# Alandroid/img-compression-mps

Measured on AMD Instinct MI355X. Metric: Mvoxels/s compress+reconstruct, 256^3 fp32, bond chi=64; SSIM vs ref, higher is better.
Workload: dtype f32

## Files before the change

### img-compression-mps_amd/csrc/gemm.hip

```cpp
#include <stdlib.h>

#include <algorithm>

#include "common.h"
#include "gemm_plan.h"

namespace {

using ndmps::f64x4;
using ndmps::load4_stream_f32;
typedef float f32x16 __attribute__((ext_vector_type(16)));

template <typename T>
struct Mfma;

template <>
struct Mfma<float> {
  static constexpr int MT = 32;
  static constexpr int KS = 2;
  static constexpr int NACC = 16;
  typedef f32x16 acc_t;
  static __device__ __forceinline__ acc_t mma(float a, float b, acc_t c) {
    return __builtin_amdgcn_mfma_f32_32x32x2f32(a, b, c, 0, 0, 0);
  }
  static __device__ __forceinline__ int acc_row(int reg, int lane) {
    return (reg & 3) + 8 * (reg >> 2) + 4 * (lane >> 5);
  }
  static __device__ __forceinline__ int acc_col(int lane) { return lane & 31; }
  static __device__ __forceinline__ int frag_idx(int lane) { return lane & 31; }
  static __device__ __forceinline__ int frag_k(int lane) { return lane >> 5; }
};

template <>
struct Mfma<double> {
  static constexpr int MT = 16;
  static constexpr int KS = 4;
  static constexpr int NACC = 4;
  typedef f64x4 acc_t;
  static __device__ __forceinline__ acc_t mma(double a, double b, acc_t c) {
    return __builtin_amdgcn_mfma_f64_16x16x4f64(a, b, c, 0, 0, 0);
  }
  static __device__ __forceinline__ int acc_row(int reg, int lane) { return (lane >> 4) + 4 * reg; }
  static __device__ __forceinline__ int acc_col(int lane) { return lane & 15; }
  static __device__ __forceinline__ int frag_idx(int lane) { return lane & 15; }
  static __device__ __forceinline__ int frag_k(int lane) { return lane >> 4; }
};

template <typename T>
struct alignas(sizeof(T) * 4) Quad {
  T v[4];
};

struct GemmIndex {
  const int64_t* a_row;
  const int64_t* a_col;
  const int64_t* c_row;
  const int64_t* c_col;
  int guarded;
};
inline int gemm_guarded_env() { return getenv("NDMPS_GEMM_GUARDED") ? 1 : 0; }

constexpr int kGemmMaxBatch = 64;
struct GemmBatchPtrs {
  const void* a[kGemmMaxBatch];
  const void* b[kGemmMaxBatch];
  void* c[kGemmMaxBatch];
};

template <typename T, int BM, int BN, int WAVES_M, int WAVES_N, bool TA, bool TB, bool VEC, bool IDX>
__device__ __forceinline__ void
gemm_body(int64_t M, int64_t N, int64_t K, const T* __restrict__ A, int64_t lda, const T* __restrict__ B, int64_t ldb,
          T* __restrict__ C, int64_t ldc, const GemmIndex& ix) {
  using MF = Mfma<T>;
  constexpr int BK = 16;
  constexpr int MT = MF::MT;
  constexpr int TM = BM / (WAVES_M * MT);
  constexpr int TN = BN / (WAVES_N * MT);
  constexpr int PAD = 4;
  constexpr int A_PER = BM * BK / 256, B_PER = BN * BK / 256;
  static_assert(WAVES_M * WAVES_N == 4, "4 waves per workgroup");
  static_assert(TM >= 1 && TN >= 1, "tile too small");
  constexpr bool VA = VEC && A_PER % 4 == 0, VB = VEC && B_PER % 4 == 0;

  __shared__ T As[BK][BM + PAD];
  __shared__ T Bs[BK][BN + PAD];

  const int tid = threadIdx.x;
  const int lane = tid & 63;
  const int wave = tid >> 6;
  const int wm = wave / WAVES_N;
  const int wn = wave % WAVES_N;
  const int64_t m0 = (int64_t)blockIdx.x * BM;
  const int64_t n0 = (int64_t)blockIdx.y * BN;

  typename MF::acc_t acc[TM][TN];
#pragma unroll
  for (int i = 0; i < TM; ++i)
#pragma unroll
    for (int j = 0; j < TN; ++j)
#pragma unroll
      for (int r = 0; r < MF::NACC; ++r) acc[i][j][r] = (T)0;

  T ra[A_PER], rb[B_PER];

  constexpr int kIdxK = 1024;
  __shared__ int64_t acol_s[(IDX && !TA && VEC) ? kIdxK : 1];
  int64_t arow_q[(A_PER / 4) > 0 ? (A_PER / 4) : 1];
  const bool idx_fast = IDX && !TA && VA && ix.a_row != nullptr && K <= kIdxK;
  if (IDX && !TA && VA) {
    if (idx_fast) {
      for (int64_t kk = tid; kk < K; kk += 256) acol_s[kk] = ix.a_col[kk];
#pragma unroll
      for (int i = 0; i < A_PER / 4; ++i) {
        const int m = (tid + 256 * i) / (BK / 4);
        arow_q[i] = m0 + m < M ? ix.a_row[m0 + m] : 0;
      }
      __syncthreads();
    }
  }

  const bool inner_a = VA && m0 + BM <= M && !ix.guarded, inner_b = VB && n0 + BN <= N && !ix.guarded;
  auto fetch_a = [&](int64_t k0) {
    if (VA && inner_a && k0 + BK <= K) {
#pragma unroll
      for (int i = 0; i < A_PER / 4; ++i) {
        const int e = tid + 256 * i;
        const T* src;
        if (TA) {
          src = A + (k0 + e / (BM / 4)) * lda + m0 + (e % (BM / 4)) * 4;
        } else {
          const int m = e / (BK / 4), k = (e % (BK / 4)) * 4;
          if (IDX && idx_fast) src = A + arow_q[i] + acol_s[k0 + k];
          else if (IDX && ix.a_row) src = A + ix.a_row[m0 + m] + ix.a_col[k0 + k];
          else src = A + (m0 + m) * lda + k0 + k;
        }
        const Quad<T> q = *reinterpret_cast<const Quad<T>*>(src);
#pragma unroll
        for (int j = 0; j < 4; ++j) ra[4 * i + j] = q.v[j];
      }
    } else if (VA) {
#pragma unroll
      for (int i = 0; i < A_PER / 4; ++i) {
        const int e = tid + 256 * i;
        Quad<T> q;
        q.v[0] = q.v[1] = q.v[2] = q.v[3] = (T)0;
        if (TA) {
          const int k = e / (BM / 4), m = (e % (BM / 4)) * 4;
          if (k0 + k < K && m0 + m < M) q = *reinterpret_cast<const Quad<T>*>(A + (k0 + k) * lda + m0 + m);
        } else {
          const int m = e / (BK / 4), k = (e % (BK / 4)) * 4;
          if (k0 + k < K && m0 + m < M) {
            if (IDX && idx_fast) q = *reinterpret_cast<const Quad<T>*>(A + arow_q[i] + acol_s[k0 + k]);
            else if (IDX && ix.a_row) q = *reinterpret_cast<const Quad<T>*>(A + ix.a_row[m0 + m] + ix.a_col[k0 + k]);
            else q = *reinterpret_cast<const Quad<T>*>(A + (m0 + m) * lda + k0 + k);
          }
        }
#pragma unroll
        for (int j = 0; j < 4; ++j) ra[4 * i + j] = q.v[j];
      }
    } else {
#pragma unroll
      for (int i = 0; i < A_PER; ++i) {
        const int e = tid + 256 * i;
        int m, k;
        if (TA) {
          k = e / BM;
          m = e % BM;
        } else {
          m = e / BK;
          k = e % BK;
        }
        const int64_t gk = k0 + k, gm = m0 + m;
        if (IDX && ix.a_row) ra[i] = (gk < K && gm < M) ? A[ix.a_row[gm] + ix.a_col[gk]] : (T)0;
        else ra[i] = (gk < K && gm < M) ? (TA ? A[gk * lda + gm] : A[gm * lda + gk]) : (T)0;
      }
    }
  };
  auto fetch_b = [&](int64_t k0) {
    if (VB && inner_b && k0 + BK <= K) {
#pragma unroll
      for (int i = 0; i < B_PER / 4; ++i) {
        const int e = tid + 256 * i;
        const T* src = TB ? B + (n0 + e / (BK / 4)) * ldb + k0 + (e % (BK / 4)) * 4
                          : B + (k0 + e / (BN / 4)) * ldb + n0 + (e % (BN / 4)) * 4;
        const Quad<T> q = *reinterpret_cast<const Quad<T>*>(src);
#pragma unroll
        for (int j = 0; j < 4; ++j) rb[4 * i + j] = q.v[j];
      }
    } else if (VB) {
#pragma unroll
      for (int i = 0; i < B_PER / 4; ++i) {
        const int e = tid + 256 * i;
        Quad<T> q;
        q.v[0] = q.v[1] = q.v[2] = q.v[3] = (T)0;
        if (TB) {
          const int n = e / (BK / 4), k = (e % (BK / 4)) * 4;
          if (k0 + k < K && n0 + n < N) q = *reinterpret_cast<const Quad<T>*>(B + (n0 + n) * ldb + k0 + k);
        } else {
          const int k = e / (BN / 4), n = (e % (BN / 4)) * 4;
          if (k0 + k < K && n0 + n < N) q = *reinterpret_cast<const Quad<T>*>(B + (k0 + k) * ldb + n0 + n);
        }
#pragma unroll
        for (int j = 0; j < 4; ++j) rb[4 * i + j] = q.v[j];
      }
    } else {
#pragma unroll
      for (int i = 0; i < B_PER; ++i) {
        const int e = tid + 256 * i;
        int n, k;
        if (TB) {
          n = e / BK;
          k = e % BK;
        } else {
          k = e / BN;
          n = e % BN;
        }
        const int64_t gk = k0 + k, gn = n0 + n;
        rb[i] = (gk < K && gn < N) ? (TB ? B[gn * ldb + gk] : B[gk * ldb + gn]) : (T)0;
      }
    }
  };
  auto commit = [&]() {
    if (VA) {
#pragma unroll
      for (int i = 0; i < A_PER / 4; ++i) {
        const int e = tid + 256 * i;
        if (TA) {
          const int k = e / (BM / 4), m = (e % (BM / 4)) * 4;
#pragma unroll
          for (int j = 0; j < 4; ++j) As[k][m + j] = ra[4 * i + j];
        } else {
          const int m = e / (BK / 4), k = (e % (BK / 4)) * 4;
#pragma unroll
          for (int j = 0; j < 4; ++j) As[k + j][m] = ra[4 * i + j];
        }
      }
    } else {
#pragma unroll
      for (int i = 0; i < A_PER; ++i) {
        const int e = tid + 256 * i;
        if (TA) As[e / BM][e % BM] = ra[i];
        else As[e % BK][e / BK] = ra[i];
      }
    }
    if (VB) {
#pragma unroll
      for (int i = 0; i < B_PER / 4; ++i) {
        const int e = tid + 256 * i;
        if (TB) {
          const int n = e / (BK / 4), k = (e % (BK / 4)) * 4;
#pragma unroll
          for (int j = 0; j < 4; ++j) Bs[k + j][n] = rb[4 * i + j];
        } else {
          const int k = e / (BN / 4), n = (e % (BN / 4)) * 4;
#pragma unroll
          for (int j = 0; j < 4; ++j) Bs[k][n + j] = rb[4 * i + j];
        }
      }
    } else {
#pragma unroll
      for (int i = 0; i < B_PER; ++i) {
        const int e = tid + 256 * i;
        if (TB) Bs[e % BK][e / BK] = rb[i];
        else Bs[e / BN][e % BN] = rb[i];
      }
    }
  };

  fetch_a(0);
  fetch_b(0);
  const int fi = MF::frag_idx(lane);
  const int fk = MF::frag_k(lane);
  for (int64_t k0 = 0; k0 < K; k0 += BK) {
    __syncthreads();
    commit();
    __syncthreads();
    if (k0 + BK < K) {
      fetch_a(k0 + BK);
      fetch_b(k0 + BK);
    }
#pragma unroll
    for (int kk = 0; kk < BK; kk += MF::KS) {
      T a[TM], b[TN];
#pragma unroll
      for (int i = 0; i < TM; ++i) a[i] = As[kk + fk][(wm * TM + i) * MT + fi];
#pragma unroll
      for (int j = 0; j < TN; ++j) b[j] = Bs[kk + fk][(wn * TN + j) * MT + fi];
#pragma unroll
      for (int i = 0; i < TM; ++i)
#pragma unroll
        for (int j = 0; j < TN; ++j) acc[i][j] = MF::mma(a[i], b[j], acc[i][j]);
    }
  }

  if constexpr (IDX && MF::MT == 32 && BM == 128 && BN == 128 && sizeof(T) == 4) {
    if (ix.c_row) {
      __shared__ float cstage[4][32][36];
      float (*st)[36] = cstage[wave];
      const int rl0 = lane >> 3, cl = (lane & 7) * 4;
      int64_t roff[TM][4], coff[TN][4];
#pragma unroll
      for (int j = 0; j < TN; ++j) {
        const int64_t col = n0 + (wn * TN + j) * MT + cl;
#pragma unroll
        for (int e = 0; e < 4; ++e) coff[j][e] = col + e < N ? ix.c_col[col + e] : -1;
      }
#pragma unroll
      for (int i = 0; i < TM; ++i)
#pragma unroll
        for (int ps = 0; ps < 4; ++ps) {
          const int64_t row = m0 + (wm * TM + i) * MT + rl0 + 8 * ps;
          roff[i][ps] = row < M ? ix.c_row[row] : -1;
        }
#pragma unroll
      for (int i = 0; i < TM; ++i)
#pragma unroll
        for (int j = 0; j < TN; ++j) {
#pragma unroll
          for (int r = 0; r < MF::NACC; ++r) st[MF::acc_row(r, lane)][MF::acc_col(lane)] = acc[i][j][r];
          __builtin_amdgcn_fence(__ATOMIC_RELEASE, "wavefront");
          __builtin_amdgcn_wave_barrier();
          __builtin_amdgcn_fence(__ATOMIC_ACQUIRE, "wavefront");
          const bool run = coff[j][0] >= 0 && coff[j][3] == coff[j][0] + 3 && coff[j][1] == coff[j][0] + 1 &&
                           coff[j][2] == coff[j][0] + 2;
#pragma unroll
          for (int ps = 0; ps < 4; ++ps) {
            const float4 v = *reinterpret_cast<const float4*>(&st[rl0 + 8 * ps][cl]);
            const int64_t ro = roff[i][ps];
            if (ro < 0) continue;
            if (run && ((ro + coff[j][0]) & 3) == 0) {
              *reinterpret_cast<float4*>(C + ro + coff[j][0]) = v;
            } else {
              if (coff[j][0] >= 0) C[ro + coff[j][0]] = v.x;
              if (coff[j][1] >= 0) C[ro + coff[j][1]] = v.y;
              if (coff[j][2] >= 0) C[ro + coff[j][2]] = v.z;
              if (coff[j][3] >= 0) C[ro + coff[j][3]] = v.w;
            }
          }
          __builtin_amdgcn_fence(__ATOMIC_RELEASE, "wavefront");
          __builtin_amdgcn_wave_barrier();
        }
      return;
    }
  }
  if (IDX && ix.c_row) {
    int64_t roff[TM][MF::NACC], coff[TN];
#pragma unroll
    for (int j = 0; j < TN; ++j) {
      const int64_t col = n0 + (wn * TN + j) * MT + MF::acc_col(lane);
      coff[j] = col < N ? ix.c_col[col] : -1;
    }
#pragma unroll
    for (int i = 0; i < TM; ++i)
#pragma unroll
      for (int r = 0; r < MF::NACC; ++r) {
        const int64_t row = m0 + (wm * TM + i) * MT + MF::acc_row(r, lane);
        roff[i][r] = row < M ? ix.c_row[row] : -1;
      }
#pragma unroll
    for (int i = 0; i < TM; ++i)
#pragma unroll
      for (int j = 0; j < TN; ++j)
#pragma unroll
        for (int r = 0; r < MF::NACC; ++r)
          if (roff[i][r] >= 0 && coff[j] >= 0) C[roff[i][r] + coff[j]] = acc[i][j][r];
    return;
  }
#pragma unroll
  for (int i = 0; i < TM; ++i)
#pragma unroll
    for (int j = 0; j < TN; ++j) {
      const int64_t col = n0 + (wn * TN + j) * MT + MF::acc_col(lane);
#pragma unroll
      for (int r = 0; r < MF::NACC; ++r) {
        const int64_t row = m0 + (wm * TM + i) * MT + MF::acc_row(r, lane);
        if (row < M && col < N) C[row * ldc + col] = acc[i][j][r];
      }
    }
}

template <typename T, int BM, int BN, int WAVES_M, int WAVES_N, bool TA, bool TB, bool VEC, bool IDX = false>
__global__ void __launch_bounds__(256, 2)
// ... 21 lines not shown
#define NDMPS_GEMM_LAUNCH(TA_, TB_, V_)                                                                            \
  do {                                                                                                              \
    if (bp)                                                                                                         \
      hipLaunchKernelGGL((gemm_batched_kernel<T, BM, BN, WAVES_M, WAVES_N, TA_, TB_, V_>), grid, block, 0, stream,  \
                         m, n, k, *bp, lda, ldb, ldc, gi);                                                          \
    else                                                                                                            \
      hipLaunchKernelGGL((gemm_kernel<T, BM, BN, WAVES_M, WAVES_N, TA_, TB_, V_>), grid, block, 0, stream, m, n, k,  \
                         A, lda, B, ldb, C, ldc, gi);                                                               \
  } while (0)
#define NDMPS_GEMM_TRANS(V_)                                     \
  do {                                                           \
    if (transA && transB) NDMPS_GEMM_LAUNCH(true, true, V_);     \
    else if (transA) NDMPS_GEMM_LAUNCH(true, false, V_);         \
    else if (transB) NDMPS_GEMM_LAUNCH(false, true, V_);         \
    else NDMPS_GEMM_LAUNCH(false, false, V_);                    \
  } while (0)
  if (plan.vec) NDMPS_GEMM_TRANS(true);
  else NDMPS_GEMM_TRANS(false);
#undef NDMPS_GEMM_TRANS
#undef NDMPS_GEMM_LAUNCH
  NDMPS_LAUNCH_CHECK();
  return NDMPS_OK;
}

template <typename T>
constexpr ndmps::GemmElem gemm_elem() {
  return sizeof(T) == 8 ? ndmps::GemmElem::F64 : ndmps::GemmElem::F32;
}

inline int64_t gemm_misalignment(const void* p) { return (int64_t)((uintptr_t)p % 64); }

template <typename T>
int gemm_check(int64_t m, int64_t n, int64_t k, const T* A, int64_t lda, int transA, const T* B,
               int64_t ldb, int transB, T* C, int64_t ldc) {
  NDMPS_REQUIRE(A && B && C, "NULL GEMM operand");
  const char* why = ndmps::gemm_refusal(gemm_elem<T>(), transA, transB, m, n, k, lda, ldb, ldc);
  NDMPS_REQUIRE(!why, "%s (m=%lld n=%lld k=%lld lda=%lld ldb=%lld ldc=%lld)", why, (long long)m, (long long)n,
                (long long)k, (long long)lda, (long long)ldb, (long long)ldc);
  return NDMPS_OK;
}

template <typename T>
int gemm_run(int transA, int transB, int64_t m, int64_t n, int64_t k, const T* A, int64_t lda, const T* B, int64_t ldb,
             T* C, int64_t ldc, ndmps_stream_t stream, const GemmBatchPtrs* bp, int batch) {
  if (bp) {
    A = static_cast<const T*>(bp->a[0]);
    B = static_cast<const T*>(bp->b[0]);
    C = static_cast<T*>(bp->c[0]);
  }
  NDMPS_TRY(gemm_check(m, n, k, A, lda, transA, B, ldb, transB, C, ldc));
  int64_t mis_a = gemm_misalignment(A), mis_b = gemm_misalignment(B), mis_c = gemm_misalignment(C);
  for (int z = 1; bp && z < batch; ++z) {
    mis_a |= gemm_misalignment(bp->a[z]);
    mis_b |= gemm_misalignment(bp->b[z]);
    mis_c |= gemm_misalignment(bp->c[z]);
  }
  const ndmps::GemmPlan plan = ndmps::gemm_plan(gemm_elem<T>(), transA, transB, m, n, k, lda, ldb, ldc, mis_a, mis_b,
                                                mis_c, gemm_guarded_env() != 0);
  if (plan.launches == 0) return NDMPS_OK;
  hipStream_t s = (hipStream_t)stream;
  if (bp) A = B = nullptr, C = nullptr;
#define NDMPS_GEMM_TILE(BM_, BN_, WM_, WN_)  \
  if (plan.bm == BM_ && plan.bn == BN_)      \
  return launch_gemm<T, BM_, BN_, WM_, WN_>(plan, transA, transB, m, n, k, A, lda, B, ldb, C, ldc, s, bp, batch)
  if constexpr (sizeof(T) == 4) {
    NDMPS_GEMM_TILE(128, 32, 4, 1);
    NDMPS_GEMM_TILE(64, 64, 2, 2);
    NDMPS_GEMM_TILE(128, 128, 2, 2);
  } else {
    NDMPS_GEMM_TILE(64, 16, 4, 1);
    NDMPS_GEMM_TILE(32, 32, 2, 2);
    NDMPS_GEMM_TILE(64, 64, 2, 2);
  }
#undef NDMPS_GEMM_TILE
  ndmps::set_error("no kernel for the planned tile %d x %d", plan.bm, plan.bn);
  return NDMPS_EINVAL;
}

int launch_gemm_indexed(const ndmps::GemmPlan& plan, int64_t m, int64_t n, int64_t k, const float* A, int64_t lda,
                        const float* B, int64_t ldb, float* C, int64_t ldc, const GemmIndex& ix, hipStream_t s,
                        const GemmBatchPtrs* bp, int batch) {
  const dim3 block(256);
  const dim3 grid((unsigned)plan.grid_x, (unsigned)plan.grid_y, (unsigned)batch);
#define NDMPS_GEMM_IDX(BM_, V_)                                                                                        \
  do {                                                                                                                  \
    if (bp)                                                                                                             \
      hipLaunchKernelGGL((gemm_batched_kernel<float, BM_, BM_, 2, 2, false, false, V_, true>), grid, block, 0, s, m, n,  \
                         k, *bp, lda, ldb, ldc, ix);                                                                    \
    else                                                                                                                \
      hipLaunchKernelGGL((gemm_kernel<float, BM_, BM_, 2, 2, false, false, V_, true>), grid, block, 0, s, m, n, k, A,    \
                         lda, B, ldb, C, ldc, ix);                                                                      \
  } while (0)
  if (plan.bm == 64) {
    if (plan.vec) NDMPS_GEMM_IDX(64, true);
    else NDMPS_GEMM_IDX(64, false);
  } else {
    if (plan.vec) NDMPS_GEMM_IDX(128, true);
    else NDMPS_GEMM_IDX(128, false);
  }
#undef NDMPS_GEMM_IDX
  NDMPS_LAUNCH_CHECK();
  return NDMPS_OK;
}

}

extern "C" int ndmps_sgemm(int transA, int transB, int64_t m, int64_t n, int64_t k, const float* d_A,
                           int64_t lda, const float* d_B, int64_t ldb, float* d_C, int64_t ldc,
                           ndmps_stream_t stream) {
  return gemm_run<float>(transA, transB, m, n, k, d_A, lda, d_B, ldb, d_C, ldc, stream, nullptr, 1);
}

extern "C" int ndmps_sgemm_indexed(int64_t m, int64_t n, int64_t k, const float* d_A, int64_t lda,
                                   const int64_t* d_a_row, const int64_t* d_a_col, int a_vec4, const float* d_B,
                                   int64_t ldb, float* d_C, int64_t ldc, const int64_t* d_c_row,
                                   const int64_t* d_c_col, ndmps_stream_t stream) {
  NDMPS_REQUIRE(m >= 0 && n >= 0 && k >= 0 && d_A && d_B && d_C, "bad indexed GEMM argument");
  NDMPS_REQUIRE((d_a_row == nullptr) == (d_a_col == nullptr) && (d_c_row == nullptr) == (d_c_col == nullptr),
                "offset tables come in (row, column) pairs");
  NDMPS_REQUIRE(ldb >= n && (d_a_row || lda >= k) && (d_c_row || ldc >= n), "leading dimension too small");
  const ndmps::GemmPlan plan = ndmps::gemm_plan_indexed(m, n, k, lda, ldb, d_a_row != nullptr, a_vec4 != 0,
                                                        gemm_misalignment(d_A), gemm_misalignment(d_B),
                                                        gemm_guarded_env() != 0);
  if (plan.launches == 0) return NDMPS_OK;
  GemmIndex ix{d_a_row, d_a_col, d_c_row, d_c_col, plan.guarded};
  return launch_gemm_indexed(plan, m, n, k, d_A, lda, d_B, ldb, d_C, ldc, ix, (hipStream_t)stream, nullptr, 1);
}

extern "C" int ndmps_dgemm(int transA, int transB, int64_t m, int64_t n, int64_t k, const double* d_A,
                           int64_t lda, const double* d_B, int64_t ldb, double* d_C, int64_t ldc,
                           ndmps_stream_t stream) {
  return gemm_run<double>(transA, transB, m, n, k, d_A, lda, d_B, ldb, d_C, ldc, stream, nullptr, 1);
}

namespace {
template <typename T>
int gemm_batched_check(int batch, const T* const* h_A, const T* const* h_B, T* const* h_C, GemmBatchPtrs& bp) {
  NDMPS_REQUIRE(batch >= 1 && batch <= kGemmMaxBatch && h_A && h_B && h_C, "batched GEMM: batch=%d outside [1, %d] or NULL array",
                batch, kGemmMaxBatch);
  for (int z = 0; z < batch; ++z) {
    NDMPS_REQUIRE(h_A[z] && h_B[z] && h_C[z], "batched GEMM: NULL operand %d", z);
    bp.a[z] = h_A[z];
    bp.b[z] = h_B[z];
    bp.c[z] = h_C[z];
  }
  return NDMPS_OK;
}
}

extern "C" int ndmps_gemm_batched_max(void) { return kGemmMaxBatch; }

extern "C" int ndmps_sgemm_batched(int batch, int transA, int transB, int64_t m, int64_t n, int64_t k,
                                   const float* const* h_A, int64_t lda, const float* const* h_B, int64_t ldb,
                                   float* const* h_C, int64_t ldc, ndmps_stream_t stream) {
  GemmBatchPtrs bp;
  NDMPS_TRY(gemm_batched_check(batch, h_A, h_B, h_C, bp));
  return gemm_run<float>(transA, transB, m, n, k, nullptr, lda, nullptr, ldb, nullptr, ldc, stream, &bp, batch);
}

extern "C" int ndmps_dgemm_batched(int batch, int transA, int transB, int64_t m, int64_t n, int64_t k,
                                   const double* const* h_A, int64_t lda, const double* const* h_B, int64_t ldb,
                                   double* const* h_C, int64_t ldc, ndmps_stream_t stream) {
  GemmBatchPtrs bp;
  NDMPS_TRY(gemm_batched_check(batch, h_A, h_B, h_C, bp));
  return gemm_run<double>(transA, transB, m, n, k, nullptr, lda, nullptr, ldb, nullptr, ldc, stream, &bp, batch);
}

extern "C" int ndmps_gemm_plan_query(int elem, int transA, int transB, int64_t m, int64_t n, int64_t k, int64_t lda,
                                     int64_t ldb, int64_t ldc, int64_t mis_a, int64_t mis_b, int64_t mis_c, int guarded,
                                     int64_t* h_out) {
  NDMPS_REQUIRE(h_out && elem >= 0 && elem <= 2, "bad GEMM plan query (elem=%d)", elem);
  NDMPS_REQUIRE(mis_a >= 0 && mis_b >= 0 && mis_c >= 0, "a misalignment is a byte count");
  const ndmps::GemmElem e = (ndmps::GemmElem)elem;
  const char* why = ndmps::gemm_refusal(e, transA, transB, m, n, k, lda, ldb, ldc);
// ... 127 lines not shown
```

### img-compression-mps_amd/csrc/tt.hip

```cpp
#include <math.h>
#include <stdlib.h>

#include <algorithm>
#include <vector>

#include "common.h"
#include "trunc.h"
#include "typed.h"

namespace {

constexpr double kCutoffFloor = 1e-6;
constexpr double kCutoffFloorF64 = 1e-8;
template <typename T>
constexpr double cutoff_floor() { return sizeof(T) == 8 ? kCutoffFloorF64 : kCutoffFloor; }
constexpr double kSweepEigTol = 1e-13;

inline double sweep_eig_tol(bool f64_storage = false) {
  const char* e = getenv("NDMPS_SWEEP_EIG_TOL");
  if (e) {
    const double v = atof(e);
    if (v >= 1e-16 && v <= 1e-6) return v;
  }
  return f64_storage ? 1e-15 : kSweepEigTol;
// ... 63 lines not shown
  const int64_t total = rows * k;
  for (int64_t e = (int64_t)blockIdx.x * 256 + threadIdx.x; e < total; e += (int64_t)gridDim.x * 256) {
    const int64_t r = e / k, c = e % k;
    const double sg = sigma[c];
    out[e] = ndmps::from_f64<T>(sg > 0.0 ? M[r * ldm + c] * pow(sg, power) : 0.0);
  }
}
template <typename T>
__device__ __forceinline__ void scale_rows_body(const double* __restrict__ M, int64_t k, int64_t n,
                                                const double* __restrict__ sigma, double power, T* __restrict__ out) {
  const int64_t total = k * n;
  for (int64_t e = (int64_t)blockIdx.x * 256 + threadIdx.x; e < total; e += (int64_t)gridDim.x * 256) {
    const double sg = sigma[e / n];
    out[e] = ndmps::from_f64<T>(sg > 0.0 ? M[e] * pow(sg, power) : 0.0);
  }
}

template <typename T>
__global__ void __launch_bounds__(256)
core_from_vectors_kernel(const double* __restrict__ V, int64_t n, int64_t k, T* __restrict__ core,
                         const int* __restrict__ rank_r, int64_t cap_r) {
  core_from_vectors_body(V, n, k, core, rank_r, cap_r);
}
template <typename T>
__global__ void __launch_bounds__(256)
scale_cols_to_f32_kernel(const double* __restrict__ M, int64_t rows, int64_t ldm, int64_t k,
                         const double* __restrict__ sigma, double power, T* __restrict__ out) {
  scale_cols_body(M, rows, ldm, k, sigma, power, out);
}
template <typename T>
__global__ void __launch_bounds__(256)
scale_rows_to_f32_kernel(const double* __restrict__ M, int64_t k, int64_t n, const double* __restrict__ sigma,
                         double power, T* __restrict__ out) {
  scale_rows_body(M, k, n, sigma, power, out);
}
__global__ void __launch_bounds__(256) sqrt_clamp_kernel(const double* __restrict__ w, int64_t n, double* s) {
  sqrt_clamp_body(w, n, s);
}

__global__ void __launch_bounds__(256)
scale_cols_sqrt_kernel(double* __restrict__ M, int64_t rows, int64_t cols, const double* __restrict__ w,
                       double rel_zero = 0.0) {
  const double zero = rel_zero * fmax(fmax(w[0], w[cols - 1]), 0.0);
  const int64_t total = rows * cols;
  for (int64_t e = (int64_t)blockIdx.x * 256 + threadIdx.x; e < total; e += (int64_t)gridDim.x * 256) {
    const double we = w[e % cols];
    M[e] *= we > zero ? sqrt(we) : 0.0;
  }
}

constexpr int kSmallBatch = 64;
struct BatchOps {
  const void* in[kSmallBatch];
  void* out[kSmallBatch];
};
template <typename T>
__global__ void __launch_bounds__(256) f32_to_f64_batched_kernel(BatchOps ops, int64_t n, double* __restrict__ y, int64_t y_stride) {
  f32_to_f64_body(static_cast<const T*>(ops.in[blockIdx.y]), n, y + (int64_t)blockIdx.y * y_stride);
}
template <typename T>
__global__ void __launch_bounds__(256)
core_from_vectors_batched_kernel(const double* __restrict__ V, int64_t v_stride, int64_t n, int64_t k, BatchOps ops,
                                 const int* __restrict__ rank_r, int64_t cap_r) {
  core_from_vectors_body(V + (int64_t)blockIdx.y * v_stride, n, k, static_cast<T*>(ops.out[blockIdx.y]),
                         rank_r ? rank_r + blockIdx.y : nullptr, cap_r);
}
__global__ void __launch_bounds__(256)
sqrt_clamp_batched_kernel(const double* __restrict__ w, int64_t stride, int64_t n, double* __restrict__ sg) {
  sqrt_clamp_body(w + (int64_t)blockIdx.y * stride, n, sg + (int64_t)blockIdx.y * stride);
}
template <typename T>
__global__ void __launch_bounds__(256)
scale_cols_to_f32_batched_kernel(const double* __restrict__ M, int64_t m_stride, int64_t rows, int64_t ldm, int64_t k,
                                 const double* __restrict__ sigma, int64_t s_stride, double power, BatchOps ops) {
  scale_cols_body(M + (int64_t)blockIdx.y * m_stride, rows, ldm, k, sigma + (int64_t)blockIdx.y * s_stride, power,
                  static_cast<T*>(ops.out[blockIdx.y]));
}
template <typename T>
__global__ void __launch_bounds__(256)
scale_rows_to_f32_batched_kernel(const double* __restrict__ M, int64_t m_stride, int64_t k, int64_t n,
                                 const double* __restrict__ sigma, int64_t s_stride, double power, BatchOps ops) {
  scale_rows_body(M + (int64_t)blockIdx.y * m_stride, k, n, sigma + (int64_t)blockIdx.y * s_stride, power,
                  static_cast<T*>(ops.out[blockIdx.y]));
}

struct MergeRanks {
  int k_right[64];
  int k_here[64];
};

__global__ void __launch_bounds__(256)
merge_stage1_kernel(const double* __restrict__ Gtop, int64_t stride_top, int n_top, const double* __restrict__ W,
                    int64_t stride_w, int ldw, double* __restrict__ T, int64_t stride_t, int n_i, int n_right,
                    int d_i, MergeRanks rk) {
  const int b = blockIdx.y;
  const int k = rk.k_right[b];
  const int cols = d_i * k;
  const double* G = Gtop + (int64_t)b * stride_top;
  const double* Wb = W + (int64_t)b * stride_w;
  double* Tb = T + (int64_t)b * stride_t;
  const int reps = n_top / n_i;
  const int64_t total = (int64_t)n_i * cols;
  for (int64_t e = (int64_t)blockIdx.x * 256 + threadIdx.x; e < total; e += (int64_t)gridDim.x * 256) {
    const int r = (int)(e / cols), col = (int)(e % cols);
    const int bb = col / k, q = col % k;
    double acc = 0.0;
    for (int t = 0; t < reps; ++t) {
      const double* grow = G + (int64_t)(t * n_i + r) * n_top + t * n_i + bb * n_right;
      for (int c = 0; c < n_right; ++c) acc = fma(grow[c], Wb[(int64_t)c * ldw + q], acc);
    }
    Tb[e] = acc;
  }
}

__global__ void __launch_bounds__(256)
merge_stage2_kernel(const double* __restrict__ T, int64_t stride_t, const double* __restrict__ W, int64_t stride_w,
                    int ldw, double* __restrict__ Gout, int64_t stride_g, int n_right, int d_i, MergeRanks rk) {
  const int b = blockIdx.y;
  const int k = rk.k_right[b];
  const int n = d_i * k;
  const double* Tb = T + (int64_t)b * stride_t;
  const double* Wb = W + (int64_t)b * stride_w;
  double* Gb = Gout + (int64_t)b * stride_g;
  const int64_t total = (int64_t)n * n;
  for (int64_t e = (int64_t)blockIdx.x * 256 + threadIdx.x; e < total; e += (int64_t)gridDim.x * 256) {
    const int row = (int)(e / n), j = (int)(e % n);
    const int a = row / k, pp = row % k;
    double acc = 0.0;
    for (int c = 0; c < n_right; ++c) acc = fma(Wb[(int64_t)c * ldw + pp], Tb[(int64_t)(a * n_right + c) * n + j], acc);
    Gb[e] = acc;
  }
}

template <typename T>
__global__ void __launch_bounds__(256)
merge_basis_kernel(const double* __restrict__ Wr, int64_t stride_w, int ldw, const double* __restrict__ V,
                   int64_t stride_v, double* __restrict__ Wout, T* __restrict__ W32, int64_t stride_w32,
                   int n_right, int d_i, MergeRanks rk) {
  const int b = blockIdx.y;
  const int kr = rk.k_right[b], kh = rk.k_here[b];
  const int n = d_i * kr;
  const double* Wb = Wr + (int64_t)b * stride_w;
  const double* Vb = V + (int64_t)b * stride_v;
  double* Ob = Wout + (int64_t)b * stride_w;
  T* O32 = W32 ? W32 + (int64_t)b * stride_w32 : nullptr;
  const int64_t total = (int64_t)d_i * n_right * kh;
  for (int64_t e = (int64_t)blockIdx.x * 256 + threadIdx.x; e < total; e += (int64_t)gridDim.x * 256) {
    const int row = (int)(e / kh), pp = (int)(e % kh);
    const int a = row / n_right, c = row % n_right;
    double acc = 0.0;
    for (int q = 0; q < kr; ++q) acc = fma(Wb[(int64_t)c * ldw + q], Vb[(int64_t)(a * kr + q) * n + pp], acc);
    Ob[(int64_t)row * ldw + pp] = acc;
    if (O32) O32[(int64_t)row * kh + pp] = ndmps::from_f64<T>(acc);
  }
}

__global__ void merge_basis_init_kernel(double* __restrict__ W, int64_t stride_w) {
  W[(int64_t)blockIdx.x * stride_w] = 1.0;
}

__global__ void __launch_bounds__(256)
gather_rows_kernel(const float* __restrict__ W, int64_t rows, int64_t cols, const int32_t* __restrict__ perm,
                   float* __restrict__ out, int64_t w_stride = 0, int64_t out_stride = 0) {
  W += (int64_t)blockIdx.y * w_stride;
  out += (int64_t)blockIdx.y * out_stride;
  const int64_t total = rows * cols;
// ... 702 lines not shown
        NDMPS_LAUNCH_CHECK();
        NDMPS_TRY(ndmps_dgemm(0, 1, m, m, n, Ab, n, Ab, n, Gb(b), m, s));
      }
    }
    return NDMPS_OK;
  }

  const int* right_ranks(int i, int base) const {
    return lay.device_rank && ws.d_ranks && i + 1 < L ? ws.d_ranks + (int64_t)(i + 1) * batch + base : nullptr;
  }

  int site_core_and_carry(int i) {
    if (uniform_small() && uniform_kept()) {
      NDMPS_TRY(core_and_carry_uniform(i));
    } else {
      for (int b = 0; b < batch; ++b) NDMPS_TRY(core_and_carry_volume(i, b));
    }
    for (int b = 0; b < batch; ++b) {
      const int64_t m = cur_elems[b] / (h_dims[i] * chi_r[b]);
      std::swap(cur[b], nxt[b]);
      cur_elems[b] = m * kept[b];
      chi_r[b] = kept[b];
      h_bonds_out[(int64_t)b * (L + 1) + i] = kept[b];
    }
    return NDMPS_OK;
  }

  int core_and_carry_uniform(int i) {
    const int64_t n = h_dims[i] * chi_r[0], m = cur_elems[0] / n, small = eig_n[0], k = kept[0];
    BatchOps cores_out, carry_out;
    std::vector<T*> pcore(batch);
    for (int b = 0; b < batch; ++b) {
      pcore[b] = core(b, i);
      cores_out.out[b] = pcore[b];
      carry_out.out[b] = nxt[b];
    }
    if (n <= m) {
      hipLaunchKernelGGL(core_from_vectors_batched_kernel<T>, dim3(grid1d(k * n), batch), dim3(256), 0, s,
                         ws.V, sq, n, k, cores_out, right_ranks(i, 0), chi_r[0]);
      NDMPS_LAUNCH_CHECK();
      int rc = NDMPS_OK;
      const bool grouped = gemm_batched_T(batch, 1, m, k, n, cur.data(), pcore.data(), n, nxt.data(), s, &rc);
      NDMPS_TRY(rc);
      for (int b = 0; b < batch && !grouped; ++b)
        NDMPS_TRY(gemm_T(1, m, k, n, cur[b], pcore[b], n, nxt[b], ws.tws, lay.transpose_bytes, s));
      return NDMPS_OK;
    }
    const auto pv = strided(ws.V, sq), pa = strided(ws.A64, lay.wide_elems), pu = strided(ws.UtA, lay.wide_elems);
    hipLaunchKernelGGL(sqrt_clamp_batched_kernel, dim3(grid1d(small), batch), dim3(256), 0, s, ws.w,
                       lay.small_max, small, ws.sig);
    hipLaunchKernelGGL(scale_cols_to_f32_batched_kernel<T>, dim3(grid1d(m * k), batch), dim3(256), 0, s, ws.V,
                       sq, m, m, k, ws.sig, lay.small_max, 1.0, carry_out);
    NDMPS_LAUNCH_CHECK();
    NDMPS_TRY(ndmps_dgemm_batched(batch, 1, 0, k, n, m, pv.data(), m, pa.data(), n, pu.data(), n, s));
    hipLaunchKernelGGL(scale_rows_to_f32_batched_kernel<T>, dim3(grid1d(k * n), batch), dim3(256), 0, s,
                       ws.UtA, lay.wide_elems, k, n, ws.sig, lay.small_max, -1.0,
                       cores_out);
    NDMPS_LAUNCH_CHECK();
    return NDMPS_OK;
  }

  int core_and_carry_volume(int i, int b) {
    const int64_t n = h_dims[i] * chi_r[b], m = cur_elems[b] / n, small = eig_n[b], k = kept[b];
    const double* sigb = ws.sig + (int64_t)b * lay.small_max;
    if (n <= m) {
      hipLaunchKernelGGL(core_from_vectors_kernel<T>, dim3(grid1d(k * n)), dim3(256), 0, s, Vb(b), n, k,
                         core(b, i), right_ranks(i, b), chi_r[b]);
      NDMPS_LAUNCH_CHECK();
      return gemm_T(1, m, k, n, cur[b], core(b, i), n, nxt[b], ws.tws, lay.transpose_bytes, s);
    }
    hipLaunchKernelGGL(sqrt_clamp_kernel, dim3(grid1d(small)), dim3(256), 0, s, ws.w + (int64_t)b * lay.small_max,
                       small, ws.sig + (int64_t)b * lay.small_max);
    hipLaunchKernelGGL(scale_cols_to_f32_kernel<T>, dim3(grid1d(m * k)), dim3(256), 0, s, Vb(b), m, m, k, sigb,
                       1.0, nxt[b]);
    NDMPS_LAUNCH_CHECK();
    NDMPS_TRY(ndmps_dgemm(1, 0, k, n, m, Vb(b), m, ws.A64 + (int64_t)b * lay.wide_elems, n, ws.UtA, n, s));
    hipLaunchKernelGGL(scale_rows_to_f32_kernel<T>, dim3(grid1d(k * n)), dim3(256), 0, s, ws.UtA, k, n, sigb,
                       -1.0, core(b, i));
    NDMPS_LAUNCH_CHECK();
    return NDMPS_OK;
  }

  int finish() {
    for (int b = 0; b < batch; ++b)
      NDMPS_CHECK_HIP(hipMemcpyAsync(core(b, 0), cur[b], cur_elems[b] * sizeof(T), hipMemcpyDeviceToDevice, s));
    if (!lay.device_rank || L <= 1) {
      if (async) {
        ndmps::set_error("an asynchronous sweep needs ranks decided on the device (ndmps_tt_sweep_pads_cores) and more than one site");
        return NDMPS_EINVAL;
      }
      NDMPS_CHECK_HIP(hipStreamSynchronize(s));
      return NDMPS_OK;
    }
    const size_t n_i = (size_t)2 * L * batch, n_s = (size_t)L * batch * lay.spec_stride;
    std::vector<int> host_i(async ? 0 : n_i);
    std::vector<double> host_s(async ? 0 : n_s);
    if (async) NDMPS_REQUIRE(async->h_ranks && (async->h_spec || n_s == 0), "asynchronous sweep without its host buffers");
    int* dst_i = async ? async->h_ranks : host_i.data();
    double* dst_s = async ? async->h_spec : host_s.data();
    NDMPS_CHECK_HIP(hipMemcpyAsync(dst_i, ws.d_ranks, n_i * sizeof(int), hipMemcpyDeviceToHost, s));
    if (n_s) NDMPS_CHECK_HIP(hipMemcpyAsync(dst_s, ws.d_spec, n_s * sizeof(double), hipMemcpyDeviceToHost, s));
    if (async) return NDMPS_OK;
    NDMPS_CHECK_HIP(hipStreamSynchronize(s));
    return sweep_collect(batch, L, lay.spec_stride, dst_i, n_s ? dst_s : nullptr, h_bonds_out, h_spectra, h_spec_offsets);
  }
};

template <typename T>
int sweep_impl(int batch, T* const* h_dense, int L, const int64_t* h_dims, double cutoff, int64_t max_bond,
               T* const* h_cores, const int64_t* h_core_offsets, int64_t* h_bonds_out, double* h_spectra,
               const int64_t* h_spec_offsets, void* d_ws, int64_t ws_bytes, ndmps_stream_t stream,
               const SweepSource* src = nullptr, const SweepAsync* async = nullptr) {
  Sweep<T> sw{batch, h_dense, L, h_dims, cutoff, max_bond, h_cores, h_core_offsets, h_bonds_out, h_spectra,
              h_spec_offsets, d_ws, ws_bytes, (hipStream_t)stream, src, async};
  NDMPS_TRY(sw.prepare());
  int i = L - 1;
  if (sw.lay.merge_from < L) {
    NDMPS_TRY(sw.merged_run());
    i = sw.lay.merge_from - 1;
  }
  for (; i >= 1; --i) {
    NDMPS_TRY(sw.site_gram(i));
    NDMPS_TRY(sw.solve_site(i, true));
    NDMPS_TRY(sw.site_core_and_carry(i));
  }
  return sw.finish();
}
}

extern "C" int ndmps_tt_sweep_pads_cores(int L, const int64_t* h_dims, int64_t max_bond) {
  SweepLayout lay;
  if (!h_dims || sweep_layout(L, h_dims, max_bond, 1, lay) != NDMPS_OK) return 0;
  return lay.device_rank ? 1 : 0;
}

extern "C" int ndmps_tt_sweep_batched_f32(int batch, float* const* h_dense, int L, const int64_t* h_dims,
                                          double cutoff, int64_t max_bond, float* const* h_cores,
                                          const int64_t* h_core_offsets, int64_t* h_bonds_out,
                                          double* h_spectra, const int64_t* h_spec_offsets, void* d_ws,
                                          int64_t ws_bytes, ndmps_stream_t stream) {
  return sweep_impl<float>(batch, h_dense, L, h_dims, cutoff, max_bond, h_cores, h_core_offsets, h_bonds_out, h_spectra,
                           h_spec_offsets, d_ws, ws_bytes, stream);
}

extern "C" int64_t ndmps_tt_merge_columns(int L, const int64_t* h_dims, int64_t max_bond) {
  SweepLayout lay;
  if (!h_dims || sweep_layout(L, h_dims, max_bond, 1, lay) != NDMPS_OK) return 0;
  if (lay.merge_from >= L || (lay.numel / lay.merge_n) * lay.merge_w > lay.numel / 2) return 0;
  if (lay.merge_n < 64 || lay.numel / lay.merge_n < 256 || lay.merge_n % 4 != 0) return 0;
  return lay.merge_n;
}

extern "C" int ndmps_tt_sweep_batched_fused_f32(int batch, const float* const* h_volume, int L, const int64_t* h_dims,
                                                double cutoff, int64_t max_bond, float* const* h_cores,
                                                const int64_t* h_core_offsets, int64_t* h_bonds_out,
                                                double* h_spectra, const int64_t* h_spec_offsets,
                                                const int64_t* d_row_off, const int64_t* d_row_off_sorted,
                                                const int32_t* d_row_order, const int64_t* d_col_off,
                                                const int32_t* d_col_perm, int64_t n_cols, void* d_ws, int64_t ws_bytes,
                                                ndmps_stream_t stream) {
  NDMPS_REQUIRE(d_row_off && d_col_off && d_col_perm && n_cols >= 1, "NULL permutation table");
  SweepSource src{d_row_off, d_row_off_sorted ? d_row_off_sorted : d_row_off, d_row_off_sorted ? d_row_order : nullptr, d_col_off,
                  d_col_perm, n_cols};
  return retry_without_team([&]() {
    return sweep_impl<float>(batch, (float* const*)h_volume, L, h_dims, cutoff, max_bond, h_cores, h_core_offsets,
                             h_bonds_out, h_spectra, h_spec_offsets, d_ws, ws_bytes, stream, &src);
  });
}
// ... 278 lines not shown
```

Measured before the change: 42540.

## Double-buffer interior indexed GEMM tiles and batch final core copies into one kernel

Adds a fast path for full interior tiles of the indexed fp32 GEMM. It double-buffers LDS with register prefetch two tiles ahead, stages the next tile in the middle of the MFMA steps, and preloads the output row/column index tables into shared memory so the epilogue can use vectorised float4 scatter when the indices are contiguous. The LDS arrays are merged into one buffer that the epilogue staging reuses, and the column-index table moves to dynamic shared memory. In tt.hip, the per-batch device-to-device memcpys in finish() are replaced by a single batched copy kernel to cut launch overhead. The changes add considerable complexity and carry risks in LDS aliasing and in the alignment assumptions.

```diff
diff --git a/img-compression-mps_amd/csrc/gemm.hip b/img-compression-mps_amd/csrc/gemm.hip
--- a/img-compression-mps_amd/csrc/gemm.hip
+++ b/img-compression-mps_amd/csrc/gemm.hip
@@ -1,6 +1,7 @@
 #include <stdlib.h>
 
 #include <algorithm>
+#include <type_traits>
 
 #include "common.h"
 #include "gemm_plan.h"
@@ -59,6 +60,10 @@
   int guarded;
 };
 inline int gemm_guarded_env() { return getenv("NDMPS_GEMM_GUARDED") ? 1 : 0; }
+constexpr int kGemmIdxK = 1024;
+inline size_t gemm_acol_bytes(const GemmIndex& ix, bool vec, int64_t k) {
+  return ix.a_row && vec && k <= kGemmIdxK ? sizeof(int64_t) * (size_t)k : 0;
+}
 
 constexpr int kGemmMaxBatch = 64;
 struct GemmBatchPtrs {
@@ -82,8 +87,18 @@
   static_assert(TM >= 1 && TN >= 1, "tile too small");
   constexpr bool VA = VEC && A_PER % 4 == 0, VB = VEC && B_PER % 4 == 0;
 
-  __shared__ T As[BK][BM + PAD];
-  __shared__ T Bs[BK][BN + PAD];
+  constexpr bool kInterior = IDX && VA && VB && !TA && !TB && sizeof(T) == 4 && MT == 32;
+  constexpr bool kPatch = IDX && MT == 32 && BM == 128 && BN == 128 && sizeof(T) == 4;
+  constexpr int NBUF = kInterior ? 2 : 1;
+  constexpr int kTileElems = NBUF * BK * (BM + PAD + BN + PAD);
+  constexpr int kPatchElems = kPatch ? 4 * 2 * 32 * 36 : 0;
+  __shared__ __attribute__((aligned(16))) T smem[kTileElems > kPatchElems ? kTileElems : kPatchElems];
+  T (*As)[BM + PAD] = reinterpret_cast<T (*)[BM + PAD]>(smem);
+  T (*Bs)[BN + PAD] = reinterpret_cast<T (*)[BN + PAD]>(smem + NBUF * BK * (BM + PAD));
+  [[maybe_unused]] int64_t* crow_s = reinterpret_cast<int64_t*>(smem + kTileElems);
+  [[maybe_unused]] int64_t* ccol_s = crow_s + BM;
+  static_assert(!kPatch || (kTileElems * sizeof(T) % 8 == 0 && kTileElems * sizeof(T) + (BM + BN / 4) * 8 <= kPatchElems * sizeof(T)),
+                "the table offsets do not fit behind the operand tiles");
 
   const int tid = threadIdx.x;
   const int lane = tid & 63;
@@ -103,8 +118,8 @@
 
   T ra[A_PER], rb[B_PER];
 
-  constexpr int kIdxK = 1024;
-  __shared__ int64_t acol_s[(IDX && !TA && VEC) ? kIdxK : 1];
+  constexpr int kIdxK = kGemmIdxK;
+  extern __shared__ int64_t acol_s[];
   int64_t arow_q[(A_PER / 4) > 0 ? (A_PER / 4) : 1];
   const bool idx_fast = IDX && !TA && VA && ix.a_row != nullptr && K <= kIdxK;
   if (IDX && !TA && VA) {
@@ -267,37 +282,205 @@
     }
   };
 
-  fetch_a(0);
-  fetch_b(0);
   const int fi = MF::frag_idx(lane);
   const int fk = MF::frag_k(lane);
-  for (int64_t k0 = 0; k0 < K; k0 += BK) {
-    __syncthreads();
-    commit();
-    __syncthreads();
-    if (k0 + BK < K) {
-      fetch_a(k0 + BK);
-      fetch_b(k0 + BK);
-    }
-#pragma unroll
-    for (int kk = 0; kk < BK; kk += MF::KS) {
-      T a[TM], b[TN];
-#pragma unroll
-      for (int i = 0; i < TM; ++i) a[i] = As[kk + fk][(wm * TM + i) * MT + fi];
-#pragma unroll
-      for (int j = 0; j < TN; ++j) b[j] = Bs[kk + fk][(wn * TN + j) * MT + fi];
-#pragma unroll
-      for (int i = 0; i < TM; ++i)
-#pragma unroll
-        for (int j = 0; j < TN; ++j) acc[i][j] = MF::mma(a[i], b[j], acc[i][j]);
-    }
-  }
-
-  if constexpr (IDX && MF::MT == 32 && BM == 128 && BN == 128 && sizeof(T) == 4) {
+
+  bool interior = false;
+  int64_t c_roff[TM][4], c_col0[TN];
+  bool c_fast = false;
+  if constexpr (kInterior) {
+    constexpr int64_t kDenseLd = (int64_t)1 << 22;
+    interior = m0 + BM <= M && n0 + BN <= N && K >= BK && K % BK == 0 && K <= kIdxK && !ix.guarded && ldb <= kDenseLd &&
+               (ix.a_row || lda <= kDenseLd);
+    if (interior) {
+      constexpr int QA = A_PER / 4, QB = B_PER / 4, STEPS = BK / MF::KS;
+      const int nt = (int)(K / BK);
+      const int kq = (tid % (BK / 4)) * 4;
+      uint32_t aoff[QA], boff[QB];
+#pragma unroll
+      for (int i = 0; i < QA; ++i) aoff[i] = (uint32_t)((((tid + 256 * i) / (BK / 4)) * lda + kq) * sizeof(T));
+#pragma unroll
+      for (int i = 0; i < QB; ++i) {
+        const int e = tid + 256 * i;
+        boff[i] = (uint32_t)(((e / (BN / 4)) * ldb + (e % (BN / 4)) * 4) * sizeof(T));
+      }
+      static_assert(!kPatch || (BM <= 256 && (BM & (BM - 1)) == 0 && ((BN / 4) & (BN / 4 - 1)) == 0), "BM, BN / 4: powers of two");
+      [[maybe_unused]] int64_t c_req_row, c_req[4];
+      if constexpr (kPatch) {
+        if (ix.c_row) {
+          c_req_row = ix.c_row[m0 + (tid & (BM - 1))];
+#pragma unroll
+          for (int e = 0; e < 4; ++e) c_req[e] = ix.c_col[n0 + (tid & (BN / 4 - 1)) * 4 + e];
+        }
+      }
+      auto park_c = [&]() {
+        if constexpr (kPatch) {
+          if (ix.c_row) {
+            if (tid < BM) crow_s[tid] = c_req_row;
+            const bool run = c_req[1] == c_req[0] + 1 && c_req[2] == c_req[0] + 2 && c_req[3] == c_req[0] + 3;
+            if (tid < BN / 4) ccol_s[tid] = run ? c_req[0] : -1;
+          }
+        }
+      };
+      Quad<T> qa[2][QA], qb[2][QB];
+      auto load = [&](auto tabled, int t, Quad<T>* a, Quad<T>* b) {
+        if constexpr (decltype(tabled)::value) {
+          const int64_t ao = acol_s[t * BK + kq];
+#pragma unroll
+          for (int i = 0; i < QA; ++i) a[i] = *reinterpret_cast<const Quad<T>*>(A + arow_q[i] + ao);
+        } else {
+          const char* at = reinterpret_cast<const char*>(A + m0 * lda + (int64_t)t * BK);
+#pragma unroll
+          for (int i = 0; i < QA; ++i) a[i] = *reinterpret_cast<const Quad<T>*>(at + aoff[i]);
+        }
+        const char* bt = reinterpret_cast<const char*>(B + (int64_t)t * BK * ldb + n0);
+#pragma unroll
+        for (int i = 0; i < QB; ++i) b[i] = *reinterpret_cast<const Quad<T>*>(bt + boff[i]);
+      };
+      constexpr int LDA_S = BM + PAD, LDB_S = BN + PAD, B_AT = NBUF * BK * LDA_S;
+      const int stage_a0 = kq * LDA_S + tid / (BK / 4);
+      const int stage_b0 = B_AT + (tid / (BN / 4)) * LDB_S + (tid % (BN / 4)) * 4;
+      const int frag_a0 = fk * LDA_S + wm * TM * MT + fi;
+      const int frag_b0 = B_AT + fk * LDB_S + wn * TN * MT + fi;
+      auto here = [](int x) {
+        asm volatile("" : "+v"(x));
+        return x;
+      };
+      auto stage = [&](int buf, const Quad<T>* a, const Quad<T>* b) {
+        const int sa = here(stage_a0 + buf * BK * LDA_S), sb = here(stage_b0 + buf * BK * LDB_S);
+#pragma unroll
+        for (int i = 0; i < QA; ++i)
+#pragma unroll
+          for (int j = 0; j < 4; ++j) smem[sa + j * LDA_S + i * (256 / (BK / 4))] = a[i].v[j];
+#pragma unroll
+        for (int i = 0; i < QB; ++i)
+#pragma unroll
+          for (int j = 0; j < 4; ++j) smem[sb + i * (256 / (BN / 4)) * LDB_S + j] = b[i].v[j];
+      };
+      auto frag = [&](int fa, int fb, int kk, T* a, T* b) {
+#pragma unroll
+        for (int i = 0; i < TM; ++i) a[i] = smem[fa + kk * LDA_S + i * MT];
+#pragma unroll
+        for (int j = 0; j < TN; ++j) b[j] = smem[fb + kk * LDB_S + j * MT];
+      };
+      auto tile = [&](auto tabled, auto parity, auto steady, int t) {
+        constexpr int P = decltype(parity)::value;
+        constexpr bool STEADY = decltype(steady)::value;
+        if (STEADY || t + 2 < nt) load(tabled, t + 2, qa[P], qb[P]);
+        T a[2][TM], b[2][TN];
+        const int fa = here(frag_a0 + P * BK * LDA_S), fb = here(frag_b0 + P * BK * LDB_S);
+        frag(fa, fb, 0, a[0], b[0]);
+#pragma unroll
+        for (int s = 0; s < STEPS; ++s) {
+          if (s + 1 < STEPS) frag(fa, fb, (s + 1) * MF::KS, a[(s + 1) & 1], b[(s + 1) & 1]);
+#pragma unroll
+          for (int i = 0; i < TM; ++i)
+#pragma unroll
+            for (int j = 0; j < TN; ++j) acc[i][j] = MF::mma(a[s & 1][i], b[s & 1][j], acc[i][j]);
+          if (s == STEPS / 2 && (STEADY || t + 1 < nt)) stage(1 - P, qa[1 - P], qb[1 - P]);
+          __builtin_amdgcn_sched_barrier(0);
+        }
+        if (STEADY || t + 1 < nt) __syncthreads();
+      };
+      using Even = std::integral_constant<int, 0>;
+      using Odd = std::integral_constant<int, 1>;
+      auto run = [&](auto tabled) {
+        load(tabled, 0, qa[0], qb[0]);
+        if (nt > 1) load(tabled, 1, qa[1], qb[1]);
+        park_c();
+        stage(0, qa[0], qb[0]);
+        __syncthreads();
+        int t = 0;
+        for (; t + 3 < nt; t += 2) {
+          tile(tabled, Even(), std::true_type(), t);
+          tile(tabled, Odd(), std::true_type(), t + 1);
+        }
+        for (; t < nt; t += 2) {
+          tile(tabled, Even(), std::false_type(), t);
+          if (t + 1 < nt) tile(tabled, Odd(), std::false_type(), t + 1);
+        }
+        if constexpr (kPatch) {
+          if (ix.c_row) {
+            const int rl0 = lane >> 3, cl = (lane & 7) * 4;
+            c_fast = true;
+#pragma unroll
+            for (int j = 0; j < TN; ++j) {
+              c_col0[j] = ccol_s[((wn * TN + j) * MT + cl) / 4];
+              c_fast = c_fast && c_col0[j] >= 0;
+            }
+#pragma unroll
+            for (int i = 0; i < TM; ++i)
+#pragma unroll
+              for (int ps = 0; ps < 4; ++ps) {
+                c_roff[i][ps] = crow_s[(wm * TM + i) * MT + rl0 + 8 * ps];
+#pragma unroll
+                for (int j = 0; j < TN; ++j) c_fast = c_fast && ((c_roff[i][ps] + c_col0[j]) & 3) == 0;
+              }
+          }
+        }
+      };
+      if (ix.a_row) run(std::true_type());
+      else run(std::false_type());
+    }
+  }
+
+  if (!interior) {
+    fetch_a(0);
+    fetch_b(0);
+    for (int64_t k0 = 0; k0 < K; k0 += BK) {
+      __syncthreads();
+      commit();
+      __syncthreads();
+      if (k0 + BK < K) {
+        fetch_a(k0 + BK);
+        fetch_b(k0 + BK);
+      }
+#pragma unroll
+      for (int kk = 0; kk < BK; kk += MF::KS) {
+        T a[TM], b[TN];
+#pragma unroll
+        for (int i = 0; i < TM; ++i) a[i] = As[kk + fk][(wm * TM + i) * MT + fi];
+#pragma unroll
+        for (int j = 0; j < TN; ++j) b[j] = Bs[kk + fk][(wn * TN + j) * MT + fi];
+#pragma unroll
+        for (int i = 0; i < TM; ++i)
+#pragma unroll
+          for (int j = 0; j < TN; ++j) acc[i][j] = MF::mma(a[i], b[j], acc[i][j]);
+      }
+    }
+  }
+
+  if constexpr (kPatch) {
     if (ix.c_row) {
-      __shared__ float cstage[4][32][36];
-      float (*st)[36] = cstage[wave];
+      __shared__ int c_ok[4];
+      const bool wave_ok = __all(c_fast);
+      if (lane == 0) c_ok[wave] = wave_ok;
+      __syncthreads();
+      float (*st)[36] = reinterpret_cast<float (*)[36]>(smem + wave * (2 * 32 * 36));
       const int rl0 = lane >> 3, cl = (lane & 7) * 4;
+      if constexpr (kInterior) {
+        if (c_ok[0] && c_ok[1] && c_ok[2] && c_ok[3]) {
+          auto put = [&](int q) {
+#pragma unroll
+            for (int r = 0; r < MF::NACC; ++r)
+              st[(q & 1) * 32 + MF::acc_row(r, lane)][MF::acc_col(lane)] = acc[q / TN][q % TN][r];
+          };
+          put(0);
+#pragma unroll
+          for (int q = 0; q < TM * TN; ++q) {
+            __builtin_amdgcn_fence(__ATOMIC_RELEASE, "wavefront");
+            __builtin_amdgcn_wave_barrier();
+            __builtin_amdgcn_fence(__ATOMIC_ACQUIRE, "wavefront");
+            float4 v[4];
+#pragma unroll
+            for (int ps = 0; ps < 4; ++ps) v[ps] = *reinterpret_cast<const float4*>(&st[(q & 1) * 32 + rl0 + 8 * ps][cl]);
+            if (q + 1 < TM * TN) put(q + 1);
+#pragma unroll
+            for (int ps = 0; ps < 4; ++ps) *reinterpret_cast<float4*>(C + c_roff[q / TN][ps] + c_col0[q % TN]) = v[ps];
+          }
+          return;
+        }
+      }
       int64_t roff[TM][4], coff[TN][4];
 #pragma unroll
       for (int j = 0; j < TN; ++j) {
@@ -485,14 +668,15 @@
                         const GemmBatchPtrs* bp, int batch) {
   const dim3 block(256);
   const dim3 grid((unsigned)plan.grid_x, (unsigned)plan.grid_y, (unsigned)batch);
-#define NDMPS_GEMM_IDX(BM_, V_)                                                                                        \
-  do {                                                                                                                  \
-    if (bp)                                                                                                             \
-      hipLaunchKernelGGL((gemm_batched_kernel<float, BM_, BM_, 2, 2, false, false, V_, true>), grid, block, 0, s, m, n,  \
-                         k, *bp, lda, ldb, ldc, ix);                                                                    \
-    else                                                                                                                \
-      hipLaunchKernelGGL((gemm_kernel<float, BM_, BM_, 2, 2, false, false, V_, true>), grid, block, 0, s, m, n, k, A,    \
-                         lda, B, ldb, C, ldc, ix);                                                                      \
+  const size_t acol = gemm_acol_bytes(ix, plan.vec != 0, k);
+#define NDMPS_GEMM_IDX(BM_, V_)                                                                                          \
+  do {                                                                                                                    \
+    if (bp)                                                                                                               \
+      hipLaunchKernelGGL((gemm_batched_kernel<float, BM_, BM_, 2, 2, false, false, V_, true>), grid, block, acol, s, m, n, \
+                         k, *bp, lda, ldb, ldc, ix);                                                                      \
+    else                                                                                                                  \
+      hipLaunchKernelGGL((gemm_kernel<float, BM_, BM_, 2, 2, false, false, V_, true>), grid, block, acol, s, m, n, k, A,   \
+                         lda, B, ldb, C, ldc, ix);                                                                        \
   } while (0)
   if (plan.bm == 64) {
     if (plan.vec) NDMPS_GEMM_IDX(64, true);
diff --git a/img-compression-mps_amd/csrc/tt.hip b/img-compression-mps_amd/csrc/tt.hip
--- a/img-compression-mps_amd/csrc/tt.hip
+++ b/img-compression-mps_amd/csrc/tt.hip
@@ -169,6 +169,16 @@
                                  const double* __restrict__ sigma, int64_t s_stride, double power, BatchOps ops) {
   scale_rows_body(M + (int64_t)blockIdx.y * m_stride, k, n, sigma + (int64_t)blockIdx.y * s_stride, power,
                   static_cast<T*>(ops.out[blockIdx.y]));
+}
+struct BatchCounts {
+  int64_t n[kSmallBatch];
+};
+template <typename T>
+__global__ void __launch_bounds__(256) copy_batched_kernel(BatchOps ops, BatchCounts counts) {
+  const T* __restrict__ x = static_cast<const T*>(ops.in[blockIdx.y]);
+  T* __restrict__ y = static_cast<T*>(ops.out[blockIdx.y]);
+  const int64_t n = counts.n[blockIdx.y];
+  for (int64_t e = (int64_t)blockIdx.x * 256 + threadIdx.x; e < n; e += (int64_t)gridDim.x * 256) y[e] = x[e];
 }
 
 struct MergeRanks {
@@ -1037,8 +1047,20 @@
   }
 
   int finish() {
-    for (int b = 0; b < batch; ++b)
-      NDMPS_CHECK_HIP(hipMemcpyAsync(core(b, 0), cur[b], cur_elems[b] * sizeof(T), hipMemcpyDeviceToDevice, s));
+    for (int base = 0; base < batch; base += kSmallBatch) {
+      const int count = std::min(kSmallBatch, batch - base);
+      BatchOps ops;
+      BatchCounts counts;
+      int64_t most = 0;
+      for (int t = 0; t < count; ++t) {
+        ops.in[t] = cur[base + t];
+        ops.out[t] = core(base + t, 0);
+        counts.n[t] = cur_elems[base + t];
+        most = std::max(most, counts.n[t]);
+      }
+      if (most > 0) hipLaunchKernelGGL(copy_batched_kernel<T>, dim3(grid1d(most), count), dim3(256), 0, s, ops, counts);
+    }
+    NDMPS_LAUNCH_CHECK();
     if (!lay.device_rank || L <= 1) {
       if (async) {
         ndmps::set_error("an asynchronous sweep needs ranks decided on the device (ndmps_tt_sweep_pads_cores) and more than one site");
```

After: 42300. Within noise of the previous version (-0.6%).
